# iSach/SoccerNeRFs

Measured on AMD Instinct MI355X. Metric: train rays/sec (K-Planes Broadcast-style, whole job), higher is better.
Workload: dtype bf16; 1 GPU; K-Planes default multiscale-res 1-16 on synthetic Broadcast-style (k-planes preset: 4096 rays/GPU/step, samples 256/128/64, 5 scales x 6 planes C=32, 156.0 M params), full train step incl. Adam; rays_per_gpu=4096, images=627, params=156049664, parallelism=single GPU

## Files before the change

include/snerf.h:

```cpp
#ifndef SNERF_H
#define SNERF_H

#include <stdint.h>

#ifdef __cplusplus
extern "C" {
#endif

typedef void* snerf_stream_t;

#define SNERF_OK 0
#define SNERF_ERR_ARG (-1)
#define SNERF_ERR_UNSUPPORTED (-2)

#define SNERF_MAX_SCALES 8
#define SNERF_ABI_VERSION 16
#define SNERF_ABI_REVISION 2

int snerf_abi_version(void);
int snerf_abi_revision(void);
const char* snerf_last_error(void);
const char* snerf_target_arch(void);

typedef struct {
// ... 221 lines not shown
} snerf_adam_dyn;
int snerf_adam_prepare(snerf_adam_dyn* dyn, float lr, float beta1, float beta2, int32_t policy, int32_t force_nonfinite, snerf_stream_t stream);

int snerf_adam_step(const float* p, float* p_out, float* g, float* m, float* v, int64_t n, float lr, float beta1, float beta2, float eps,
                    int32_t step, float grad_scale, int32_t zero_grad, snerf_adam_dyn* dyn, snerf_stream_t stream);

int snerf_adam_planes_step(const snerf_kplanes_desc* desc, const float* p_in, float* p_out, float* g, float* m, float* v,
                           float c_space_tv, float c_time_smooth, float c_sparse, float* losses, int32_t n_slots, float lr, float beta1,
                           float beta2, float eps, int32_t step, float grad_scale, int32_t zero_grad, snerf_adam_dyn* dyn,
                           snerf_stream_t stream);

int snerf_adam_planes_step_range(const snerf_kplanes_desc* desc, const float* p_in, float* p_out, float* g, float* m, float* v,
                                 float c_space_tv, float c_time_smooth, float c_sparse, float* losses, int32_t n_slots, float lr, float beta1,
                                 float beta2, float eps, int32_t step, float grad_scale, int32_t zero_grad, int64_t range_lo, int64_t range_hi,
                                 snerf_adam_dyn* dyn, snerf_stream_t stream);

#define SNERF_COMM_ID_BYTES 128
int snerf_comm_unique_id(void* id128);
int snerf_comm_create(int32_t world, int32_t rank, const void* id128, void** comm_out);
int snerf_comm_destroy(void* comm);
int snerf_allreduce_grads(void* comm, float* grads, int64_t n, snerf_stream_t stream);


typedef struct {
  const int64_t* indices;
  const float* fx; const float* fy; const float* cx; const float* cy;
  const float* c2w;
  const float* cam_times;
  int32_t R;
  int32_t collide;
// ... 152 lines not shown
                                float* target, snerf_stream_t stream);

int snerf_sample_pixels_sphere(const float* u, int32_t R, int32_t M, int32_t H, int32_t W, const uint8_t* images, int64_t* indices,
                               float* target, snerf_stream_t stream);

int snerf_mask_pack(const uint8_t* mask, int64_t n_pixels, int64_t first_pixel, int64_t count, uint32_t* bits, int32_t* block_counts,
                    snerf_stream_t stream);

int snerf_sample_pixels_masked(const float* u, int32_t R, int32_t M, int32_t H, int32_t W, const uint32_t* bits, const int64_t* block_prefix,
                               int64_t n_blocks, const uint8_t* images, int64_t* indices, float* target, snerf_stream_t stream);

int snerf_sort_rays_by_key(const int64_t* indices_in, const int32_t* image_key, int32_t n_keys, int32_t R, const float* aux_in, int32_t aux_cols,
                           int64_t* indices_out, float* aux_out, snerf_stream_t stream);

int snerf_ray_time_order(const float* times, int32_t R, int32_t* order_out, snerf_stream_t stream);

int snerf_aabb_collide(const float* origins, const float* dirs, int32_t R, const float* aabb6, float near_plane, int32_t training,
                       float* nears, float* fars, snerf_stream_t stream);

typedef struct {
  int32_t D;
  int32_t C;
  int32_t L;
  int32_t grid_C;
  int32_t H;
  int32_t gridtype;
  int32_t align_corners;
  float S;
  int32_t offsets[33];
} snerf_tgrid_desc;
// ... 142 lines not shown
```

soccernerfs_amd/_lib.py:

```python
import ctypes as C
import os

import torch

_PKG = os.path.dirname(os.path.abspath(__file__))
LIB_PATH = os.path.join(_PKG, "libsnerf.so")

MAX_SCALES = 8
ABI_VERSION = 16
ABI_REVISION = 2


class KPlanesDesc(C.Structure):
    _c_struct_ = "snerf_kplanes_desc"
    _fields_ = [
        ("n_scales", C.c_int32),
        ("C", C.c_int32),
        ("concat", C.c_int32),
        ("n_coords", C.c_int32),
        ("res", (C.c_int32 * 4) * MAX_SCALES),
        ("off", (C.c_int64 * 6) * MAX_SCALES),
    ]


# ... 30 lines not shown
    _c_struct_ = "snerf_mlp_desc"
    _fields_ = [("d_in", C.c_int32), ("hidden", C.c_int32), ("n_hidden", C.c_int32), ("d_out", C.c_int32),
                ("hidden_act", C.c_int32), ("out_act", C.c_int32), ("operands", C.c_int32)]


class DensityBwdLevel(C.Structure):
    _c_struct_ = "snerf_density_bwd_level"
    _fields_ = [("desc", C.c_void_p), ("planes", C.c_void_p), ("coords", C.c_void_p), ("N", C.c_int64), ("net", C.c_void_p), ("W", C.c_void_p),
                ("gdens", C.c_void_p), ("grad_planes", C.c_void_p), ("workspace", C.c_void_p), ("gX", C.c_void_p)]


class AdamDyn(C.Structure):
    _c_struct_ = "snerf_adam_dyn"
    _fields_ = [("nonfinite", C.c_int32), ("t", C.c_int32), ("skipped", C.c_int32), ("dropped", C.c_int32),
                ("step_size", C.c_float), ("inv_sqrt_bc2", C.c_float), ("skip", C.c_int32), ("_pad", C.c_int32)]


class RenderArgs(C.Structure):
    _c_struct_ = "snerf_render_args"
    _fields_ = [("weights", C.c_void_p), ("rgb", C.c_void_p), ("ebins", C.c_void_p), ("bg", C.c_void_p),
                ("R", C.c_int32), ("S", C.c_int32), ("bg_mode", C.c_int32), ("training", C.c_int32),
                ("rgb_out", C.c_void_p), ("acc_out", C.c_void_p), ("depth_median", C.c_void_p), ("depth_expected", C.c_void_p),
                ("median_rgb", C.c_void_p), ("median_index", C.c_void_p)]


class RayTrainArgs(C.Structure):
    _c_struct_ = "snerf_ray_train_args"
    _fields_ = [("density", C.c_void_p), ("ebins", C.c_void_p), ("sbins", C.c_void_p), ("rgb", C.c_void_p), ("bg", C.c_void_p), ("target", C.c_void_p),
                ("R", C.c_int32), ("S", C.c_int32), ("bg_mode", C.c_int32), ("go_scale", C.c_float), ("dist_scale", C.c_float),
                ("weights", C.c_void_p), ("rgb_out", C.c_void_p), ("acc_out", C.c_void_p), ("depth_median", C.c_void_p), ("sqerr_rays", C.c_void_p),
# ... 120 lines not shown
    "snerf_kplanes_density_bwd": "s:PIP",
    "snerf_kplanes_density_bwd_budget": "s:PIIP",
    "snerf_render_fwd": "s:PP",
    "snerf_ray_train_fwd_bwd": "s:PP",
    "snerf_render_bwd": "s:PPPIPPIIPPIP",
    "snerf_render_mse_bwd": "s:PPPIPPFIIPPPP",
    "snerf_distortion": "s:PPIIFPPIP",
    "snerf_interlevel": "s:PPIPPIIFPPP",
    "snerf_depth_loss": "s:PPPPFIIFPPIP",
    "snerf_urf_depth_loss": "s:PPPPPFIIFPPPIP",
    "snerf_plane_reg": "s:PPPFFFPIIP",
    "snerf_adam_prepare": "s:PFFFIIP",
    "snerf_adam_step": "s:PPPPPLFFFFIFIPP",
    "snerf_adam_planes_step": "s:PPPPPPFFFPIFFFFIFIPP",
    "snerf_adam_planes_step_range": "s:PPPPPPFFFPIFFFFIFILLPP",
    "snerf_comm_unique_id": "s:P",
    "snerf_comm_create": "s:IIPP",
    "snerf_comm_destroy": "s:P",
    "snerf_allreduce_grads": "s:PPLP",
    "snerf_raygen": "s:PP",
    "snerf_raygen_frame": "s:PP",
    "snerf_raygen_lens": "s:PP",
    "snerf_raygen_frame_lens": "s:PP",
    "snerf_raygen_cam": "s:PP",
    "snerf_raygen_frame_cam": "s:PP",
    "snerf_pose_apply": "s:PPPIIPP",
    "snerf_raygen_pose_bwd": "s:PP",
    "snerf_sample_pixels_uniform": "s:PIIIIPPPP",
    "snerf_sample_pixels_sphere": "s:PIIIIPPPP",
    "snerf_mask_pack": "s:PLLLPPP",
    "snerf_sample_pixels_masked": "s:PIIIIPPLPPPP",
    "snerf_sort_rays_by_key": "s:PPIIPIPPP",
    "snerf_ray_time_order": "s:PIPP",
    "snerf_aabb_collide": "s:PPIPFIPPP",
    "snerf_tgrid_encode_fwd": "s:PPPPPILPP",
    "snerf_tgrid_encode_fwd_dydx": "s:PPPPPILPPP",
    "snerf_tgrid_input_bwd": "s:PPLIIIPP",
    "snerf_tgrid_encode_bwd": "s:PPPPILPPP",
    "snerf_tgrid_encode_bwd_fx": "s:PPPPILPPP",
    "snerf_tgrid_tile_plan_make": "s:PLIIP",
    "snerf_tgrid_bwd_bin": "s:PPPPILPPPPPP",
    "snerf_tgrid_bwd_tiles": "s:PPLPPPPPP",
    "snerf_tgrid_bwd_tiles_adam": "s:PPLPPPPPPPPFFFFIIIPP",
    "snerf_tgrid_encode_bwd_levels": "s:PPPPILPPIIP",
    "snerf_tgrid_tv_fwd": "s:PLIIIPIP",
    "snerf_tgrid_tv_bwd": "s:PLIIIPPP",
    "snerf_tgrid_tv_fwd_bwd": "s:PLIIIFPIPP",
    "snerf_tgrid_tv_sign": "s:PLIIIFPIPP",
# ... 92 lines not shown
```

soccernerfs_amd/csrc/optim.hip:

```cpp
#include "plane_adam_common.hpp"

namespace snerf {

__global__ void adam_prepare_kernel(snerf_adam_dyn* dyn, float lr, float b1, float b2, int policy, int force_nonfinite) {
  if (threadIdx.x != 0 || blockIdx.x != 0) return;
  const int nf = dyn->nonfinite | force_nonfinite;
  const int skip = (policy == 1 && nf) ? 1 : 0;
  dyn->nonfinite = 0;
  dyn->skip = skip;
  if (skip) { dyn->skipped += 1; return; }
  const int t = dyn->t + 1;
  dyn->t = t;
  const double bc1 = 1.0 - pow((double)b1, (double)t), bc2 = 1.0 - pow((double)b2, (double)t);
  dyn->step_size = (float)((double)lr / bc1);
  dyn->inv_sqrt_bc2 = (float)(1.0 / sqrt(bc2));
}

template <int C, bool ADAM>
__global__ __launch_bounds__(256) void plane_reg_kernel(RegArgs a) {
  int s = 0, p = 0;
  const int blk = (int)blockIdx.x + a.blk_base;
  {
    const int b = blk;
    bool found = false;
    for (int ss = a.d.n_scales - 1; ss >= 0 && !found; --ss)
      for (int pp = a.n_planes - 1; pp >= 0; --pp)
        if (b >= a.blk_off[ss][pp]) { s = ss; p = pp; found = true; break; }
  }
  int ax, bx;
  plane_axes(a.n_planes, p, ax, bx);
  const int W = a.d.res[s][ax], H = a.d.res[s][bx];
  const bool time_plane = (a.n_planes == 6) && (bx == 3);
  constexpr int C4 = C / 4;
  const uint32_t n4 = (uint32_t)H * (uint32_t)W * C4;
  const uint32_t e = (uint32_t)(blk - a.blk_off[s][p]) * 256u + threadIdx.x;
  float l_tv = 0.f, l_sm = 0.f, l_l1 = 0.f;
// ... 32 lines not shown
        *reinterpret_cast<float4*>(gp) = add4(old, g);
      }
    }
  }
  __shared__ float red[3][4];
  l_tv = wave_sum(l_tv); l_sm = wave_sum(l_sm); l_l1 = wave_sum(l_l1);
  const int wv = threadIdx.x >> 6, lane = threadIdx.x & 63;
  if (lane == 0) { red[0][wv] = l_tv; red[1][wv] = l_sm; red[2][wv] = l_l1; }
  __syncthreads();
  if (threadIdx.x < 3 && a.losses) {
    float v = red[threadIdx.x][0] + red[threadIdx.x][1] + red[threadIdx.x][2] + red[threadIdx.x][3];
    if (v != 0.f) atomicAdd(a.losses + (size_t)(blk % a.n_slots) * 16 + threadIdx.x, v);
  }
}

__global__ __launch_bounds__(256) void adam_kernel(const float* p, float* p_out, float* __restrict__ g, float* __restrict__ m, float* __restrict__ v,
                                                  int64_t n, float step_size_h, float b1, float b2, float inv_sqrt_bc2_h, float eps,
                                                  float grad_scale, int zero_grad, snerf_adam_dyn* dyn) {
  const int64_t n4 = n / 4;
  const int64_t i = (int64_t)blockIdx.x * blockDim.x + threadIdx.x;
  const DynConsts dc = load_dyn(dyn, step_size_h, inv_sqrt_bc2_h);
  const float step_size = dc.step_size, inv_sqrt_bc2 = dc.inv_sqrt_bc2;
  if (dc.skip) {
    if (i < n4) {
      if (p_out != p) stnt4(p_out + i * 4, ldnt4(p + i * 4));
      if (zero_grad) stnt4(g + i * 4, make_float4(0.f, 0.f, 0.f, 0.f));
    }
    if (blockIdx.x == 0 && threadIdx.x < (n & 3)) {
      const int64_t j = n4 * 4 + threadIdx.x;
      p_out[j] = p[j];
      if (zero_grad) g[j] = 0.f;
    }
    return;
  }
  if (i < n4) {
    float4 pp = ldnt4(p + i * 4), gg = ldnt4(g + i * 4), mm = ldnt4(m + i * 4), vv = ldnt4(v + i * 4);
    float* P = &pp.x; float* G = &gg.x; float* M = &mm.x; float* V = &vv.x;
    int ndrop = 0;
#pragma unroll
    for (int k = 0; k < 4; ++k) {
      float gk = G[k] * grad_scale;
      if (!(fabsf(gk) <= 3.402823466e+38f)) { gk = 0.f; ++ndrop; }
      M[k] = b1 * M[k] + (1.f - b1) * gk;
      V[k] = b2 * V[k] + (1.f - b2) * gk * gk;
      float denom = sqrtf(V[k]) * inv_sqrt_bc2 + eps;
      P[k] = P[k] - step_size * (M[k] / denom);
    }
    if (ndrop && dyn) atomicAdd(&dyn->dropped, ndrop);
    stnt4(p_out + i * 4, pp);
    stnt4(m + i * 4, mm);
    stnt4(v + i * 4, vv);
    if (zero_grad && (gg.x != 0.f || gg.y != 0.f || gg.z != 0.f || gg.w != 0.f)) stnt4(g + i * 4, make_float4(0.f, 0.f, 0.f, 0.f));
  }
  if (blockIdx.x == 0 && threadIdx.x < (n & 3)) {
    int64_t i = n4 * 4 + threadIdx.x;
    float gk = g[i] * grad_scale;
    if (!(fabsf(gk) <= 3.402823466e+38f)) { gk = 0.f; if (dyn) atomicAdd(&dyn->dropped, 1); }
    float mk = b1 * m[i] + (1.f - b1) * gk;
    float vk = b2 * v[i] + (1.f - b2) * gk * gk;
    m[i] = mk; v[i] = vk;
    p_out[i] = p[i] - step_size * (mk / (sqrtf(vk) * inv_sqrt_bc2 + eps));
    if (zero_grad) g[i] = 0.f;
  }
}

__global__ __launch_bounds__(256) void adam_tv_kernel(float* p, float* __restrict__ g, float* __restrict__ m, float* __restrict__ v, int64_t n, float step_size_h,
                                                     float b1, float b2, float inv_sqrt_bc2_h, float eps, float grad_scale, int zero_grad, int grid_C, int col_a,
                                                     int col_b, const float* __restrict__ srow, snerf_adam_dyn* dyn) {
  const int64_t n4 = n / 4;
  const int64_t i = (int64_t)blockIdx.x * blockDim.x + threadIdx.x;
  if (i >= n4) return;
  const DynConsts dc = load_dyn(dyn, step_size_h, inv_sqrt_bc2_h);
  const float step_size = dc.step_size, inv_sqrt_bc2 = dc.inv_sqrt_bc2;
  if (dc.skip) {
    if (zero_grad) stnt4(g + i * 4, make_float4(0.f, 0.f, 0.f, 0.f));
    return;
  }
// ... 106 lines not shown
  if (desc->C == 32) hipLaunchKernelGGL((plane_reg_kernel<32, true>), dim3(grid), dim3(256), 0, st, a);
  else if (desc->C == 16) hipLaunchKernelGGL((plane_reg_kernel<16, true>), dim3(grid), dim3(256), 0, st, a);
  else hipLaunchKernelGGL((plane_reg_kernel<8, true>), dim3(grid), dim3(256), 0, st, a);
  SNERF_LAUNCH_CHECK("adam_planes_step");
  return 0;
}

extern "C" int snerf_adam_planes_step(const snerf_kplanes_desc* desc, const float* p_in, float* p_out, float* g, float* m, float* v,
                                      float c_space_tv, float c_time_smooth, float c_sparse, float* losses, int32_t n_slots, float lr, float beta1,
                                      float beta2, float eps, int32_t step, float grad_scale, int32_t zero_grad, snerf_adam_dyn* dyn,
                                      snerf_stream_t stream) {
  return snerf_adam_planes_step_range(desc, p_in, p_out, g, m, v, c_space_tv, c_time_smooth, c_sparse, losses, n_slots, lr, beta1, beta2, eps, step,
                                      grad_scale, zero_grad, 0, INT64_MAX & ~(int64_t)3, dyn, stream);
}

extern "C" int snerf_adam_step_tv(float* p, float* g, float* m, float* v, int64_t rows, int32_t grid_C, int32_t col_a, int32_t col_b, const float* srow,
                                  float lr, float beta1, float beta2, float eps, int32_t step, float grad_scale, int32_t zero_grad, snerf_adam_dyn* dyn,
                                  snerf_stream_t stream) {
  SNERF_REQUIRE(rows >= 1 && grid_C >= 4 && (step >= 1 || dyn), "adam_step_tv: rows=%lld grid_C=%d step=%d", (long long)rows, grid_C, step);
  SNERF_REQUIRE(col_a >= 0 && col_a < grid_C && col_b >= 0 && col_b < grid_C && col_a != col_b, "adam_step_tv: columns (%d, %d) of %d", col_a, col_b, grid_C);
  SNERF_REQUIRE(p && g && m && v && srow, "adam_step_tv: null buffer");
  const int64_t n = rows * grid_C;
  SNERF_REQUIRE((n & 3) == 0, "adam_step_tv: rows * grid_C = %lld must be a multiple of 4", (long long)n);
  SNERF_REQUIRE((((uintptr_t)p | (uintptr_t)g | (uintptr_t)m | (uintptr_t)v) & 15) == 0, "adam_step_tv: buffers must be 16-byte aligned");
  float step_size = 0.f, inv_sqrt_bc2 = 0.f;
  if (!dyn) adam_consts(lr, beta1, beta2, step, step_size, inv_sqrt_bc2);
  const int64_t blocks = (n / 4 + 255) / 256;
  SNERF_REQUIRE(blocks < (1LL << 31), "adam_step_tv: table too large for one launch");
  hipLaunchKernelGGL(adam_tv_kernel, dim3((unsigned)blocks), dim3(256), 0, (hipStream_t)stream, p, g, m, v, n, step_size, beta1, beta2, inv_sqrt_bc2, eps,
                     grad_scale, zero_grad, grid_C, col_a, col_b, srow, dyn);
// ... 30 lines not shown
```

soccernerfs_amd/csrc/raygen.hip:

```cpp
#include "raygen_common.hpp"

#pragma clang fp contract(off)

namespace snerf {

struct RaygenArgs {
  const int64_t* indices;
  const float* fx; const float* fy; const float* cx; const float* cy;
  const float* c2w;
  const float* cam_times;
  int R;
  float* origins; float* dirs; float* pixel_area; float* dir_norm; float* times;
  int collide; int training; float near_plane;
  float aabb_min[3], aabb_max[3];
  float* nears; float* fars;
};

__global__ void raygen_kernel(RaygenArgs a) {
  int r = blockIdx.x * blockDim.x + threadIdx.x;
  if (r >= a.R) return;
  const int64_t c = a.indices[(int64_t)r * 3], yi = a.indices[(int64_t)r * 3 + 1], xi = a.indices[(int64_t)r * 3 + 2];
  const PixelRay p = pixel_ray(yi, xi, a.fx[c], a.fy[c], a.cx[c], a.cy[c], a.c2w + c * 12);
#pragma unroll
  for (int k = 0; k < 3; ++k) { a.origins[(int64_t)r * 3 + k] = p.o[k]; a.dirs[(int64_t)r * 3 + k] = p.d[k]; }
// ... 112 lines not shown
  for (int i = threadIdx.x; i < n_pow2; i += blockDim.x)
    s_tk[i] = i < R ? (((uint64_t)__float_as_uint(times[i]) << 32) | (uint32_t)i) : ~0ull;
  __syncthreads();
  for (int k = 2; k <= n_pow2; k <<= 1)
    for (int lj = 31 - __clz(k >> 1); lj >= 0; --lj) {
      const int j = 1 << lj;
      for (int t = threadIdx.x; t < n_pow2 / 2; t += blockDim.x) {
        const int i = ((t >> lj) << (lj + 1)) | (t & (j - 1)), l = i + j;
        const bool up = (i & k) == 0;
        const uint64_t a = s_tk[i], b = s_tk[l];
        if ((a > b) == up) { s_tk[i] = b; s_tk[l] = a; }
      }
      __syncthreads();
    }
  for (int r = threadIdx.x; r < R; r += blockDim.x) order_out[r] = (int32_t)(uint32_t)s_tk[r];
}

__global__ void aabb_kernel(const float* __restrict__ o, const float* __restrict__ d, int R, float near_plane, int training, const float* amin3,
                            float* __restrict__ nears, float* __restrict__ fars, float a0, float a1, float a2, float b0, float b1, float b2) {
  int r = blockIdx.x * blockDim.x + threadIdx.x;
  if (r >= R) return;
  const float mn[3] = {a0, a1, a2}, mx[3] = {b0, b1, b2};
  float tn = -INFINITY, tf = INFINITY;
#pragma unroll
  for (int k = 0; k < 3; ++k) {
    float inv = 1.f / (d[(int64_t)r * 3 + k] + 1e-6f);
    float t1 = (mn[k] - o[(int64_t)r * 3 + k]) * inv, t2 = (mx[k] - o[(int64_t)r * 3 + k]) * inv;
    tn = fmaxf(tn, fminf(t1, t2));
    tf = fminf(tf, fmaxf(t1, t2));
  }
// ... 214 lines not shown
extern "C" int snerf_sort_rays_by_key(const int64_t* indices_in, const int32_t* image_key, int32_t n_keys, int32_t R, const float* aux_in,
                                      int32_t aux_cols, int64_t* indices_out, float* aux_out, snerf_stream_t stream) {
  SNERF_REQUIRE(R >= 0 && R <= 16384 && n_keys >= 1 && n_keys <= (1 << 18) && aux_cols >= 0,
                "sort_rays_by_key: R=%d (<= 16384) n_keys=%d (<= 262144) aux_cols=%d", R, n_keys, aux_cols);
  if (R == 0) return 0;
  SNERF_REQUIRE(indices_in && image_key && indices_out && indices_in != indices_out && (aux_cols == 0 || (aux_in && aux_out && aux_in != aux_out)),
                "sort_rays_by_key: null or aliased buffer (the sort is out of place)");
  int n = 2;
  while (n < R) n <<= 1;
  hipLaunchKernelGGL(sort_rays_kernel, dim3(1), dim3(256), (size_t)n * sizeof(uint32_t), (hipStream_t)stream, indices_in, image_key, R, n, aux_in, aux_cols,
                     indices_out, aux_out);
  SNERF_LAUNCH_CHECK("sort_rays_by_key");
  return 0;
}

extern "C" int snerf_ray_time_order(const float* times, int32_t R, int32_t* order_out, snerf_stream_t stream) {
  SNERF_REQUIRE(R >= 0 && R <= 16384, "ray_time_order: R=%d (<= 16384: one workgroup sorts in LDS)", R);
  if (R == 0) return 0;
  SNERF_REQUIRE(times && order_out, "ray_time_order: null buffer");
  int n = 2;
  while (n < R) n <<= 1;
  SNERF_ALLOW_LDS(ray_time_order_kernel, 16384 * (int)sizeof(uint64_t));
  hipLaunchKernelGGL(ray_time_order_kernel, dim3(1), dim3(256), (size_t)n * sizeof(uint64_t), (hipStream_t)stream, times, R, n, order_out);
  SNERF_LAUNCH_CHECK("ray_time_order");
  return 0;
}

extern "C" int snerf_aabb_collide(const float* origins, const float* dirs, int32_t R, const float* aabb6, float near_plane, int32_t training,
                                  float* nears, float* fars, snerf_stream_t stream) {
  SNERF_REQUIRE(R >= 0 && aabb6, "aabb_collide: bad arguments");
  if (R == 0) return 0;
  SNERF_REQUIRE(origins && dirs && nears && fars, "aabb_collide: null buffer");
  hipLaunchKernelGGL(aabb_kernel, dim3(ceil_div(R, 256)), dim3(256), 0, (hipStream_t)stream, origins, dirs, R, near_plane, training, nullptr, nears,
                     fars, aabb6[0], aabb6[1], aabb6[2], aabb6[3], aabb6[4], aabb6[5]);
  SNERF_LAUNCH_CHECK("aabb_collide");
  return 0;
}

extern "C" int snerf_pose_apply(const float* c2w, const float* pose_adjustment, const int32_t* group, int32_t M, int32_t G, float* c2w_adj,
                                snerf_stream_t stream) {
// ... 32 lines not shown
```

soccernerfs_amd/ops.py:

```python
import ctypes as C

from typing import Optional

import torch

from . import _lib
from .plane_set import PlaneSet


def _stream():
    return C.c_void_p(torch.cuda.current_stream().cuda_stream)


def _ptr(t: torch.Tensor):
    return C.c_void_p(t.data_ptr())


def _f32c(t: torch.Tensor, name: str) -> torch.Tensor:
    if not t.is_cuda:
        raise RuntimeError(f"{name}: expected a HIP device tensor (the HIP library is the only product path)")
    if t.dtype != torch.float32:
        raise RuntimeError(f"{name}: expected float32, got {t.dtype}")
    return t.contiguous()

# ... 828 lines not shown
    R = indices.shape[0]
    if R > 16384 or R == 0:
        return (indices, aux) if aux is not None else indices
    if not indices.is_cuda or indices.dtype != torch.int64 or image_key.dtype != torch.int32 or not image_key.is_cuda:
        raise RuntimeError("sort_rays_by_time: indices must be an int64 HIP tensor [R,3] and image_key an int32 HIP tensor")
    indices = indices.contiguous()
    out = torch.empty_like(indices)
    aux_c = _f32c(aux, "sort_rays_by_time aux").reshape(R, -1) if aux is not None else None
    aux_out = torch.empty_like(aux_c) if aux_c is not None else None
    _lib.call("sort_rays_by_key", _ptr(indices), _ptr(image_key), n_keys, R, _ptr(aux_c) if aux_c is not None else None,
              aux_c.shape[1] if aux_c is not None else 0, _ptr(out), _ptr(aux_out) if aux_out is not None else None,
              _stream())
    return (out, aux_out.view(aux.shape)) if aux is not None else out


def ray_time_order(times: torch.Tensor, out: Optional[torch.Tensor] = None) -> torch.Tensor:
    times = _f32c(times, "times").reshape(-1)
    R = times.numel()
    if out is None:
        out = torch.empty(R, dtype=torch.int32, device=times.device)
    if not out.is_cuda or out.dtype != torch.int32 or not out.is_contiguous() or out.numel() < R:
        raise RuntimeError("ray_time_order: out must be a contiguous int32 HIP tensor of at least R elements")
    _lib.call("ray_time_order", _ptr(times), R, _ptr(out), _stream())
    return out[:R]


def sample_pixels_uniform(u: torch.Tensor, num_images: int, height: int, width: int, images: Optional[torch.Tensor] = None):
    u = _f32c(u, "u")
    R = u.shape[0]
    idx = torch.empty(R, 3, dtype=torch.int64, device=u.device)
    target = None
    if images is not None:
        if not images.is_cuda or images.dtype != torch.uint8 or not images.is_contiguous() or tuple(images.shape) != (num_images, height, width, 3):
            raise RuntimeError("sample_pixels_uniform: images must be a contiguous uint8 HIP tensor [M,H,W,3]")
        target = torch.empty(R, 3, dtype=torch.float32, device=u.device)
    _lib.call("sample_pixels_uniform", _ptr(u), R, num_images, height, width, _ptr(images) if images is not None else None, _ptr(idx),
              _ptr(target) if target is not None else None, _stream())
    return idx, target
# ... 111 lines not shown
```

soccernerfs_amd/trainer.py:

```python
import ctypes as C
from dataclasses import dataclass, field
from typing import Dict, List, Optional, Sequence, Tuple

import torch

from . import _lib, ops
from .fused_step import FusedStep, _On, _align4, anneal_value, cosine_lr_factor, update_schedule
from .streams import side_stream
from .plane_set import PlaneSet
from .tcnn_compat import Network


@dataclass
class KPlanesTrainConfig:

    aabb_scale: float = 1.5
    spacetime_resolution: Sequence[int] = (64, 64, 64, 100)
    multiscale_res: Sequence[int] = (1, 2, 4, 8, 16)
    feature_dim: int = 32
    proposal_resolutions: Sequence[Sequence[int]] = ((128, 128, 128, 100), (256, 256, 256, 100))
    proposal_feature_dim: int = 8
    sigma_net_hidden_dim: int = 128
    rgb_net_hidden_dim: int = 64
    disable_viewing_dependent: bool = True
# ... 34 lines not shown
    mlp_grad_workspace: bool = True
    interleave_proposal_levels: bool = False
    fix_capacity: Optional[int] = None
    exchange_chunks: int = 2
    grad_transport: str = "fp32"
    param_transport: str = "fp32"
    emulate_transports: str = ""
    deterministic: bool = False
    nonfinite_policy: str = "skip_step"
    fused_field: bool = True
    quotient_scatter: bool = True
    quotient_epilogue: bool = True
    fused_proposal: bool = True
    fused_proposal_backward: bool = True
    proposal_backward_workgroups_per_cu: float = 1.0
    pass_b_beside_head: bool = True
    sort_before_field_fwd: bool = False
    field_fwd_time_order: bool = True
    pipeline_sweep: str = ""
    ray_gradients: bool = False
    freeze_time_planes: bool = False
    freeze_space_planes: bool = False


class KPlanesTrainer(FusedStep):

    def __init__(self, cfg: KPlanesTrainConfig, num_rays: int, device="cuda:0", process_group=None):
        self.cfg, self.R, self.dev = cfg, num_rays, torch.device(device)
        self.pg = process_group
        self.world = torch.distributed.get_world_size(process_group) if process_group is not None else 1
# ... 159 lines not shown
        self.pass_b_beside_head = cfg.pass_b_beside_head
        self._in_train_step = False
        self.fused_proposal = bool(cfg.fused_proposal and all(self.lib.snerf_kplanes_density_fwd_supported(C.byref(dp), C.byref(net.desc))
                                                             for dp, net in zip(self._desc_prop, self.prop_nets)))
        self._keep_pfeat = True
        self.fused_proposal_backward = bool(cfg.fused_proposal_backward and self.fused_proposal and not cfg.deterministic
                                            and all(f"prop{i}.mlp" in self._mlp_ws for i in range(len(self.prop_nets)))
                                            and all(self.lib.snerf_kplanes_density_bwd_supported(C.byref(dp), C.byref(net.desc))
                                                    for dp, net in zip(self._desc_prop, self.prop_nets)))
        if cfg.proposal_backward_workgroups_per_cu < 0:
            raise ValueError(f"proposal_backward_workgroups_per_cu={cfg.proposal_backward_workgroups_per_cu} (0 = uncapped, or workgroups per CU)")
        self._prop_bwd_workgroups = 0
        if cfg.proposal_backward_workgroups_per_cu > 0 and self.fused_proposal_backward:
            cus = torch.cuda.get_device_properties(self.dev).multi_processor_count
            self._prop_bwd_workgroups = max(1, int(round(cfg.proposal_backward_workgroups_per_cu * cus)))
        if self.world > 1:
            self._plan_exchange()

    @torch.no_grad()
    def _sync_frozen_halves(self):
        if self._frozen:
            self._params_alt.copy_(self.params)

    def _plain_adam_ranges(self):
        if not self._frozen:
            return [(0, self.n_proposal_params, "proposal_networks"), (self.n_proposal_params, self.n_params, "fields")]
        out = []
        sets = [(f"prop{i}.planes", ps, "proposal_networks") for i, ps in enumerate(self.prop_planes)] + [("field.planes", self.field_planes, "fields")]
        for name, ps, g in sets:
            o = self.off[name][0]
# ... 424 lines not shown
                proposal_chain(after=main.record_event())
        if not overlap:
            self._proposal_backward(proposal_grads)
        self._prop_pending = None
        for st in joins:
            if defer_prop_join and not sharded and st is self._side.get("prop"):
                self._prop_pending = st
            else:
                main.wait_stream(st)
        if cfg.ray_gradients:
            self._ray_gradient(self._desc_field, self.field_planes.planes, self._coords[2], R * self.S[2], b["gfeat"])
        self._reduce_mlp_grads(("field.sigma", "field.color"))
        if self._prop_pending is None:
            self._reduce_mlp_grads(("prop0.mlp", "prop1.mlp"))

    def _join_prop(self):
        if self._prop_pending is not None:
            torch.cuda.current_stream().wait_stream(self._prop_pending)
            self._prop_pending = None
            self._reduce_mlp_grads(("prop0.mlp", "prop1.mlp"))

    def loss_dict(self) -> Dict[str, torch.Tensor]:
        b, co, R = self.buf, self.cfg.loss_coefficients, self.R
        self._join_prop()
        if self._reg_work is not None:
            self._reg_work.wait()
        if self._field_adam_done is not None:
            torch.cuda.current_stream().wait_event(self._field_adam_done)
        d = dict(self.last)
        d["rgb_loss"] = b["sqerr"].sum() / (3 * R) * co["rgb_loss"]
        d["distortion_loss"] = b["dist_rays"].mean() * co["distortion_loss"]
        d["interlevel_loss"] = (b["inter_rays"][0].sum() + b["inter_rays"][1].sum()) / (R * self.S[2]) * co["interlevel_loss"]
        reg = b["reg"][:, :, :3].sum(1)
        d["space_tv_loss"], d["time_smoothness_loss"], d["sparse_transients_loss"] = (
            reg[0, 0] * co["space_tv_loss"], reg[0, 1] * co["time_smoothness_loss"], reg[0, 2] * co["sparse_transients_loss"])
# ... 166 lines not shown
        self._reg_work = sdist.all_reduce_sum_(self.buf["reg"][0], self.pg, async_op=True)
        self._params_alt = self.params
        self._repoint(new)
        self._finish_step()

    def _adam_mlps(self, new, off, lr, gs):
        with self._span("adam_step.mlps"):
            o0, n0 = off["field.sigma"]
            o1, n1 = off["field.color"]
            dyn_f, dyn_p = self._dyn["fields"], self._dyn["proposal_networks"]
            for (o, n), dyn in ((off["prop0.mlp"], dyn_p), (off["prop1.mlp"], dyn_p), ((o0, o1 + n1 - o0), dyn_f)):
                n4 = _align4(n)
                ops.adam_step(self.params[o:o + n4], self.grads[o:o + n4], self.exp_avg[o:o + n4], self.exp_avg_sq[o:o + n4], self.step + 1, lr,
                              eps=self.cfg.adam_eps, grad_scale=gs, zero_grad=True, p_out=new[o:o + n4], dyn=dyn)

    def _finest_offset(self) -> int:
        return int(self._desc_field.off[len(self.cfg.multiscale_res) - 1][0])

    def _adam_field_range(self, lo: int, hi: Optional[int], side: bool, role: str = "adam", span: str = "adam_planes.field", after=None):
        cfg, co = self.cfg, self.cfg.loss_coefficients
        lr = cfg.lr * cosine_lr_factor(self.step, cfg.warm_up_end, cfg.max_steps, cfg.lr_alpha)
        n4 = _align4(self.field_planes.numel)
        rng_ = (lo, n4 if hi is None else hi)
        o, n = self.off["field.planes"]
        args = (self.field_planes, self.params[o:o + n], self._params_alt[o:o + n], self.gviews["field.planes"], self.mviews["field.planes"],
                self.vviews["field.planes"], tuple(co[k] for k in ("space_tv_loss", "time_smoothness_loss", "sparse_transients_loss")),
                self.buf["reg"][0], self.step + 1, lr)
        self._prepare_group("fields", lr)
        kw = dict(eps=cfg.adam_eps, grad_scale=self._grad_scale, zero_grad=True, shard_range=rng_, dyn=self._dyn["fields"], desc=self._desc_field)
        if not side:
# ... 27 lines not shown
        if self.grads_fx is not None:
            self._join_prop()
            self._convert_fx()
        if not fused_reg:
            self._join_prop()
            self._prepare_group("fields", lr)
            self._prepare_group("proposal_networks", lr)
            with self._span("adam_step"):
                for lo, hi, g in self._plain_adam_ranges():
                    ops.adam_step(self.params[lo:hi], self.grads[lo:hi], self.exp_avg[lo:hi], self.exp_avg_sq[lo:hi], self.step + 1, lr, eps=cfg.adam_eps,
                                  grad_scale=gs, zero_grad=True, dyn=self._dyn[g])
            self._finish_step()
            return
        new = self._params_alt
        off = self.off
        sl = lambda t, name: t[off[name][0]:off[name][0] + off[name][1]]
        async_field = self.async_field_adam and self.overlap
        if not self._reg_zeroed:
            self.buf["reg"].zero_()
        emu = self.cfg.emulate_transports if self.world == 1 else ""
        if emu in ("grad", "both"):
            gv = self.gviews["field.planes"]
            gv.copy_(gv.to(torch.bfloat16))
        if async_field and self._passb_fine_done is not None:
            cut = self._finest_offset()
            ev, fine_first = self._passb_fine_done
            first, second = ((cut, None), (0, cut)) if fine_first else ((0, cut), (cut, None))
            names = ("adam_planes.field.fine", "adam_planes.field.coarse") if fine_first else ("adam_planes.field.coarse", "adam_planes.field.fine")
            self._adam_field_range(*first, side=True, role="sort", after=ev, span=names[0])
            fine_done = self._stream("sort").record_event()
            self._adam_field_range(*second, side=True, span=names[1])
            self._stream("adam").wait_event(fine_done)
            self._passb_fine_done = None
            self.field_sweep_launches = 2
        else:
            self._passb_fine_done = None
            self._adam_field_range(0, None, side=async_field)
            self.field_sweep_launches = 1
        if emu in ("param", "both"):
            o_, n_ = self.off["field.planes"]
            with _On(self, self._stream("adam") if async_field else torch.cuda.current_stream()):
                old_, new_ = self.params[o_:o_ + n_], self._params_alt[o_:o_ + n_]
                new_.copy_(old_ + (new_ - old_).to(torch.bfloat16).float())
        if async_field:
            self._field_adam_done = self._stream("adam").record_event()
        self._reg_zeroed = False
        self._join_prop()
        self._prepare_group("fields", lr)
        self._prepare_group("proposal_networks", lr)
        sets = [(f"prop{i}.planes", self.prop_planes[i], ("space_tv_proposal_loss", "time_smoothness_proposal_loss",
                                                          "sparse_transients_proposal_loss"), 1 + i) for i in range(2)]
        for name, ps, keys, row in sets:
            with self._span("adam_planes." + name.split(".")[0]):
                ops.adam_planes_step(ps, sl(self.params, name), sl(new, name), self.gviews[name], self.mviews[name], self.vviews[name],
                                     tuple(co[k] for k in keys), self.buf["reg"][row], self.step + 1, lr, eps=cfg.adam_eps, grad_scale=gs,
                                     dyn=self._dyn["proposal_networks"], desc=self._desc_prop[row - 1])
        self._adam_mlps(new, off, lr, gs)
        self._params_alt = self.params
        self._repoint(new)
        self._finish_step()

    def random_draws(self) -> Dict[str, torch.Tensor]:
        R, (S0, S1, S2) = self.R, self.S
        sj = self.cfg.use_single_jitter
        c0, c1, c2 = (1, 1, 1) if sj else (S0 + 1, S1 + 1, S2 + 1)
        flat = torch.rand(R * (c0 + c1 + c2 + 3), device=self.dev)
        o = 0
        out = []
        for c in (c0, c1, c2, 3):
            out.append(flat[o:o + R * c].view(R, c))
            o += R * c
        return {"t_rand": out[0], "u": [out[1], out[2]], "bg": out[3]}

    def train_step(self, rays: Dict[str, torch.Tensor], target: torch.Tensor, rng: Optional[Dict[str, torch.Tensor]] = None,
                   depth: Optional[torch.Tensor] = None):
# ... 109 lines not shown
```

Measured before the change: 2.166 million rays/s.

## Fuse proposal-plane and MLP Adam updates into one segmented launch; rank-based ray time order

Adds a segmented Adam kernel that updates both proposal plane sets (with their regularizer terms) and the flat MLP parameter ranges in a single launch. It also folds the replicated MLP gradient workspace into the gradient inside the Adam pass instead of running a separate reduction. Separately, the single-workgroup bitonic sort for ray time ordering is replaced with a multi-workgroup counting-rank kernel. The aim is to cut kernel launch count and serial tail work in the optimizer phase. The cost is more complex segment bookkeeping and O(R^2) comparisons for the ranking.

```diff
diff --git a/include/snerf.h b/include/snerf.h
--- a/include/snerf.h
+++ b/include/snerf.h
@@ -259,6 +259,26 @@
                                  float c_space_tv, float c_time_smooth, float c_sparse, float* losses, int32_t n_slots, float lr, float beta1,
                                  float beta2, float eps, int32_t step, float grad_scale, int32_t zero_grad, int64_t range_lo, int64_t range_hi,
                                  snerf_adam_dyn* dyn, snerf_stream_t stream);
+
+typedef struct {
+  int32_t kind;
+  int32_t n_slots;
+  const snerf_kplanes_desc* desc;
+  const float* p_in;
+  float* p_out;
+  float* g;
+  float* m;
+  float* v;
+  float c_space_tv, c_time_smooth, c_sparse;
+  int32_t _pad;
+  float* losses;
+  int64_t n;
+  snerf_adam_dyn* dyn;
+  const snerf_mlp_desc* net;
+  float* workspace;
+} snerf_adam_segment;
+int snerf_adam_segments_step(const snerf_adam_segment* segs, int32_t n_segs, float lr, float beta1, float beta2, float eps, int32_t step,
+                             float grad_scale, int32_t zero_grad, snerf_stream_t stream);
 
 #define SNERF_COMM_ID_BYTES 128
 int snerf_comm_unique_id(void* id128);
@@ -441,6 +461,7 @@
                            int64_t* indices_out, float* aux_out, snerf_stream_t stream);
 
 int snerf_ray_time_order(const float* times, int32_t R, int32_t* order_out, snerf_stream_t stream);
+int snerf_ray_time_order_reference(const float* times, int32_t R, int32_t* order_out, snerf_stream_t stream);
 
 int snerf_aabb_collide(const float* origins, const float* dirs, int32_t R, const float* aabb6, float near_plane, int32_t training,
                        float* nears, float* fars, snerf_stream_t stream);
diff --git a/soccernerfs_amd/_lib.py b/soccernerfs_amd/_lib.py
--- a/soccernerfs_amd/_lib.py
+++ b/soccernerfs_amd/_lib.py
@@ -68,6 +68,13 @@
     _c_struct_ = "snerf_adam_dyn"
     _fields_ = [("nonfinite", C.c_int32), ("t", C.c_int32), ("skipped", C.c_int32), ("dropped", C.c_int32),
                 ("step_size", C.c_float), ("inv_sqrt_bc2", C.c_float), ("skip", C.c_int32), ("_pad", C.c_int32)]
+
+
+class AdamSegment(C.Structure):
+    _c_struct_ = "snerf_adam_segment"
+    _fields_ = [("kind", C.c_int32), ("n_slots", C.c_int32), ("desc", C.c_void_p), ("p_in", C.c_void_p), ("p_out", C.c_void_p), ("g", C.c_void_p),
+                ("m", C.c_void_p), ("v", C.c_void_p), ("c_space_tv", C.c_float), ("c_time_smooth", C.c_float), ("c_sparse", C.c_float),
+                ("_pad", C.c_int32), ("losses", C.c_void_p), ("n", C.c_int64), ("dyn", C.c_void_p), ("net", C.c_void_p), ("workspace", C.c_void_p)]
 
 
 class RenderArgs(C.Structure):
@@ -218,6 +225,7 @@
     "snerf_adam_step": "s:PPPPPLFFFFIFIPP",
     "snerf_adam_planes_step": "s:PPPPPPFFFPIFFFFIFIPP",
     "snerf_adam_planes_step_range": "s:PPPPPPFFFPIFFFFIFILLPP",
+    "snerf_adam_segments_step": "s:PIFFFFIFIP",
     "snerf_comm_unique_id": "s:P",
     "snerf_comm_create": "s:IIPP",
     "snerf_comm_destroy": "s:P",
@@ -236,6 +244,7 @@
     "snerf_sample_pixels_masked": "s:PIIIIPPLPPPP",
     "snerf_sort_rays_by_key": "s:PPIIPIPPP",
     "snerf_ray_time_order": "s:PIPP",
+    "snerf_ray_time_order_reference": "s:PIPP",
     "snerf_aabb_collide": "s:PPIPFIPPP",
     "snerf_tgrid_encode_fwd": "s:PPPPPILPP",
     "snerf_tgrid_encode_fwd_dydx": "s:PPPPPILPPP",
diff --git a/soccernerfs_amd/csrc/optim.hip b/soccernerfs_amd/csrc/optim.hip
--- a/soccernerfs_amd/csrc/optim.hip
+++ b/soccernerfs_amd/csrc/optim.hip
@@ -1,3 +1,4 @@
+#include "mlp_args.hpp"
 #include "plane_adam_common.hpp"
 
 namespace snerf {
@@ -17,9 +18,8 @@
 }
 
 template <int C, bool ADAM>
-__global__ __launch_bounds__(256) void plane_reg_kernel(RegArgs a) {
+__device__ __forceinline__ void plane_reg_block(const RegArgs& a, const int blk) {
   int s = 0, p = 0;
-  const int blk = (int)blockIdx.x + a.blk_base;
   {
     const int b = blk;
     bool found = false;
@@ -82,22 +82,52 @@
   }
 }
 
-__global__ __launch_bounds__(256) void adam_kernel(const float* p, float* p_out, float* __restrict__ g, float* __restrict__ m, float* __restrict__ v,
-                                                  int64_t n, float step_size_h, float b1, float b2, float inv_sqrt_bc2_h, float eps,
-                                                  float grad_scale, int zero_grad, snerf_adam_dyn* dyn) {
+template <int C, bool ADAM>
+__global__ __launch_bounds__(256) void plane_reg_kernel(RegArgs a) {
+  plane_reg_block<C, ADAM>(a, (int)blockIdx.x + a.blk_base);
+}
+
+struct FlatFold { float* ws; int64_t ws_stride, n_fold; int reps; };
+template <bool FOLD>
+__device__ __forceinline__ float fold_gw(const FlatFold& f, int64_t e, float g, bool& folded) {
+  if (!FOLD || e >= f.n_fold) return g;
+  float s = 0.f;
+  for (int k = 0; k < f.reps; ++k) {
+    s += f.ws[k * f.ws_stride + e];
+    f.ws[k * f.ws_stride + e] = 0.f;
+  }
+  if (s != 0.f) { g = g + s; folded = true; }
+  return g;
+}
+
+template <bool FOLD>
+__device__ __forceinline__ void adam_flat_block(const float* p, float* p_out, float* __restrict__ g, float* __restrict__ m, float* __restrict__ v,
+                                                int64_t n, float step_size_h, float b1, float b2, float inv_sqrt_bc2_h, float eps, float grad_scale,
+                                                int zero_grad, snerf_adam_dyn* dyn, const FlatFold& fold, const int64_t blk) {
   const int64_t n4 = n / 4;
-  const int64_t i = (int64_t)blockIdx.x * blockDim.x + threadIdx.x;
+  const int64_t i = blk * blockDim.x + threadIdx.x;
   const DynConsts dc = load_dyn(dyn, step_size_h, inv_sqrt_bc2_h);
   const float step_size = dc.step_size, inv_sqrt_bc2 = dc.inv_sqrt_bc2;
   if (dc.skip) {
     if (i < n4) {
       if (p_out != p) stnt4(p_out + i * 4, ldnt4(p + i * 4));
+      if (FOLD && i * 4 < fold.n_fold) {
+        float4 gg = ldnt4(g + i * 4);
+        float* G = &gg.x;
+        bool folded = false;
+#pragma unroll
+        for (int k = 0; k < 4; ++k) G[k] = fold_gw<FOLD>(fold, i * 4 + k, G[k], folded);
+        if (!zero_grad && folded) stnt4(g + i * 4, gg);
+      }
       if (zero_grad) stnt4(g + i * 4, make_float4(0.f, 0.f, 0.f, 0.f));
     }
-    if (blockIdx.x == 0 && threadIdx.x < (n & 3)) {
+    if (blk == 0 && threadIdx.x < (n & 3)) {
       const int64_t j = n4 * 4 + threadIdx.x;
       p_out[j] = p[j];
+      bool folded = false;
+      const float gj = fold_gw<FOLD>(fold, j, g[j], folded);
       if (zero_grad) g[j] = 0.f;
+      else if (folded) g[j] = gj;
     }
     return;
   }
@@ -105,8 +135,10 @@
     float4 pp = ldnt4(p + i * 4), gg = ldnt4(g + i * 4), mm = ldnt4(m + i * 4), vv = ldnt4(v + i * 4);
     float* P = &pp.x; float* G = &gg.x; float* M = &mm.x; float* V = &vv.x;
     int ndrop = 0;
+    bool folded = false;
 #pragma unroll
     for (int k = 0; k < 4; ++k) {
+      G[k] = fold_gw<FOLD>(fold, i * 4 + k, G[k], folded);
       float gk = G[k] * grad_scale;
       if (!(fabsf(gk) <= 3.402823466e+38f)) { gk = 0.f; ++ndrop; }
       M[k] = b1 * M[k] + (1.f - b1) * gk;
@@ -119,16 +151,57 @@
     stnt4(m + i * 4, mm);
     stnt4(v + i * 4, vv);
     if (zero_grad && (gg.x != 0.f || gg.y != 0.f || gg.z != 0.f || gg.w != 0.f)) stnt4(g + i * 4, make_float4(0.f, 0.f, 0.f, 0.f));
-  }
-  if (blockIdx.x == 0 && threadIdx.x < (n & 3)) {
+    else if (FOLD && folded) stnt4(g + i * 4, gg);
+  }
+  if (blk == 0 && threadIdx.x < (n & 3)) {
     int64_t i = n4 * 4 + threadIdx.x;
-    float gk = g[i] * grad_scale;
+    bool folded = false;
+    const float gi = fold_gw<FOLD>(fold, i, g[i], folded);
+    float gk = gi * grad_scale;
     if (!(fabsf(gk) <= 3.402823466e+38f)) { gk = 0.f; if (dyn) atomicAdd(&dyn->dropped, 1); }
     float mk = b1 * m[i] + (1.f - b1) * gk;
     float vk = b2 * v[i] + (1.f - b2) * gk * gk;
     m[i] = mk; v[i] = vk;
     p_out[i] = p[i] - step_size * (mk / (sqrtf(vk) * inv_sqrt_bc2 + eps));
     if (zero_grad) g[i] = 0.f;
+    else if (folded) g[i] = gi;
+  }
+}
+
+__global__ __launch_bounds__(256) void adam_kernel(const float* p, float* p_out, float* __restrict__ g, float* __restrict__ m, float* __restrict__ v,
+                                                  int64_t n, float step_size_h, float b1, float b2, float inv_sqrt_bc2_h, float eps,
+                                                  float grad_scale, int zero_grad, snerf_adam_dyn* dyn) {
+  adam_flat_block<false>(p, p_out, g, m, v, n, step_size_h, b1, b2, inv_sqrt_bc2_h, eps, grad_scale, zero_grad, dyn, FlatFold{}, (int64_t)blockIdx.x);
+}
+
+constexpr int SEG_PLANE_SETS = 2, SEG_FLAT = 4;
+struct FlatSeg {
+  const float* p; float* p_out; float* g; float* m; float* v;
+  int64_t n;
+  snerf_adam_dyn* dyn;
+  FlatFold fold;
+};
+struct SegArgs {
+  RegArgs plane[SEG_PLANE_SETS];
+  FlatSeg flat[SEG_FLAT];
+  int first[SEG_PLANE_SETS + SEG_FLAT];
+  int n_plane, n_flat;
+  float step_size, b1, b2, inv_sqrt_bc2, eps, grad_scale;
+  int zero_grad;
+};
+
+template <int C>
+__global__ __launch_bounds__(256) void adam_segments_kernel(SegArgs a) {
+  const int b = (int)blockIdx.x;
+  int seg = 0;
+  for (int k = 1; k < a.n_plane + a.n_flat; ++k)
+    if (b >= a.first[k]) seg = k;
+  if (seg < a.n_plane) {
+    plane_reg_block<C, true>(a.plane[seg], b - a.first[seg]);
+  } else {
+    const FlatSeg& f = a.flat[seg - a.n_plane];
+    adam_flat_block<true>(f.p, f.p_out, f.g, f.m, f.v, f.n, a.step_size, a.b1, a.b2, a.inv_sqrt_bc2, a.eps, a.grad_scale, a.zero_grad, f.dyn, f.fold,
+                          (int64_t)(b - a.first[seg]));
   }
 }
 
@@ -265,6 +338,79 @@
                                       grad_scale, zero_grad, 0, INT64_MAX & ~(int64_t)3, dyn, stream);
 }
 
+extern "C" int snerf_adam_segments_step(const snerf_adam_segment* segs, int32_t n_segs, float lr, float beta1, float beta2, float eps, int32_t step,
+                                        float grad_scale, int32_t zero_grad, snerf_stream_t stream) {
+  SNERF_REQUIRE(segs && n_segs >= 1 && n_segs <= SEG_PLANE_SETS + SEG_FLAT, "adam_segments_step: %d segments (1..%d)", n_segs, SEG_PLANE_SETS + SEG_FLAT);
+  SegArgs a = {};
+  a.b1 = beta1; a.b2 = beta2; a.eps = eps; a.grad_scale = grad_scale; a.zero_grad = zero_grad;
+  int C = 0;
+  bool need_step = false;
+  int64_t grid[SEG_PLANE_SETS + SEG_FLAT];
+  int64_t plane_blocks[SEG_PLANE_SETS];
+  for (int k = 0; k < n_segs; ++k) {
+    const snerf_adam_segment& g = segs[k];
+    SNERF_REQUIRE(g.kind == 0 || g.kind == 1, "adam_segments_step: segment %d has kind %d (0 flat, 1 plane set)", k, g.kind);
+    SNERF_REQUIRE(g.p_in && g.p_out && g.g && g.m && g.v, "adam_segments_step: segment %d: null buffer", k);
+    need_step = need_step || !g.dyn;
+    if (g.kind == 1) {
+      const snerf_kplanes_desc* desc = g.desc;
+      SNERF_REQUIRE(a.n_plane < SEG_PLANE_SETS, "adam_segments_step: more than %d plane sets", SEG_PLANE_SETS);
+      SNERF_REQUIRE(desc && g.p_in != g.p_out, "adam_segments_step: segment %d: a plane set needs its descriptor and ping-pong parameters (p_in != p_out)", k);
+      SNERF_REQUIRE(desc->n_scales >= 1 && desc->n_scales <= SNERF_MAX_SCALES, "adam_segments_step: n_scales=%d", desc->n_scales);
+      SNERF_REQUIRE(desc->C == 8 || desc->C == 16 || desc->C == 32, "adam_segments_step: C=%d unsupported", desc->C);
+      SNERF_REQUIRE(C == 0 || C == desc->C, "adam_segments_step: the plane sets of one call share a channel count (%d, %d)", C, desc->C);
+      SNERF_REQUIRE(desc->n_coords == 3 || desc->n_coords == 4, "adam_segments_step: n_coords=%d", desc->n_coords);
+      SNERF_REQUIRE(!g.losses || g.n_slots >= 1, "adam_segments_step: n_slots=%d", g.n_slots);
+      C = desc->C;
+      RegArgs& r = a.plane[a.n_plane];
+      r.d = *desc;
+      r.n_planes = desc->n_coords == 4 ? 6 : 3;
+      r.planes = g.p_in; r.grad = g.g; r.c_tv = g.c_space_tv; r.c_smooth = g.c_time_smooth; r.c_l1 = g.c_sparse; r.losses = g.losses; r.n_slots = g.n_slots;
+      r.p_out = g.p_out; r.m = g.m; r.v = g.v; r.b1 = beta1; r.b2 = beta2; r.eps = eps; r.grad_scale = grad_scale; r.zero_grad = zero_grad;
+      r.range_lo = 0; r.range_hi = INT64_MAX & ~(int64_t)3; r.dyn = g.dyn; r.blk_base = 0;
+      int64_t blocks = 0;
+      for (int sc = 0; sc < desc->n_scales; ++sc)
+        for (int pl = 0; pl < r.n_planes; ++pl) {
+          int ax, bx;
+          plane_axes(r.n_planes, pl, ax, bx);
+          r.blk_off[sc][pl] = (int)blocks;
+          blocks += ((int64_t)desc->res[sc][ax] * desc->res[sc][bx] * (desc->C / 4) + 255) / 256;
+        }
+      plane_blocks[a.n_plane++] = blocks;
+    } else {
+      SNERF_REQUIRE(a.n_flat < SEG_FLAT, "adam_segments_step: more than %d flat segments", SEG_FLAT);
+      SNERF_REQUIRE(g.n >= 1, "adam_segments_step: segment %d: n=%lld", k, (long long)g.n);
+      SNERF_REQUIRE((((uintptr_t)g.p_in | (uintptr_t)g.p_out | (uintptr_t)g.g | (uintptr_t)g.m | (uintptr_t)g.v) & 15) == 0,
+                    "adam_segments_step: segment %d: buffers must be 16-byte aligned", k);
+      FlatSeg& f = a.flat[a.n_flat];
+      f.p = g.p_in; f.p_out = g.p_out; f.g = g.g; f.m = g.m; f.v = g.v; f.n = g.n; f.dyn = g.dyn;
+      if (g.net || g.workspace) {
+        SNERF_REQUIRE(g.net && g.workspace, "adam_segments_step: segment %d: a workspace to fold needs its MLP descriptor, and the other way round", k);
+        const int64_t n_fold = snerf_mlp_param_count(g.net);
+        SNERF_REQUIRE(n_fold > 0 && n_fold <= g.n, "adam_segments_step: segment %d: the net has %lld weights, the segment %lld floats", k, (long long)n_fold,
+                      (long long)g.n);
+        f.fold.ws = g.workspace; f.fold.ws_stride = gw_ws_stride(g.net); f.fold.n_fold = n_fold; f.fold.reps = GW_REPLICAS;
+      }
+      grid[SEG_PLANE_SETS + a.n_flat++] = ((g.n + 3) / 4 + 255) / 256;
+    }
+  }
+  SNERF_REQUIRE(!need_step || step >= 1, "adam_segments_step: step=%d (1-based) for a segment without device-side state", step);
+  if (need_step) adam_consts(lr, beta1, beta2, step, a.step_size, a.inv_sqrt_bc2);
+  for (int k = 0; k < a.n_plane; ++k) { a.plane[k].step_size = a.step_size; a.plane[k].inv_sqrt_bc2 = a.inv_sqrt_bc2; }
+  int64_t blocks = 0;
+  for (int k = 0; k < a.n_plane + a.n_flat; ++k) {
+    a.first[k] = (int)blocks;
+    blocks += k < a.n_plane ? plane_blocks[k] : grid[SEG_PLANE_SETS + k - a.n_plane];
+    SNERF_REQUIRE(blocks < (1LL << 31), "adam_segments_step: too many workgroups");
+  }
+  hipStream_t st = (hipStream_t)stream;
+  if (C == 32) hipLaunchKernelGGL((adam_segments_kernel<32>), dim3((unsigned)blocks), dim3(256), 0, st, a);
+  else if (C == 16) hipLaunchKernelGGL((adam_segments_kernel<16>), dim3((unsigned)blocks), dim3(256), 0, st, a);
+  else hipLaunchKernelGGL((adam_segments_kernel<8>), dim3((unsigned)blocks), dim3(256), 0, st, a);
+  SNERF_LAUNCH_CHECK("adam_segments_step");
+  return 0;
+}
+
 extern "C" int snerf_adam_step_tv(float* p, float* g, float* m, float* v, int64_t rows, int32_t grid_C, int32_t col_a, int32_t col_b, const float* srow,
                                   float lr, float beta1, float beta2, float eps, int32_t step, float grad_scale, int32_t zero_grad, snerf_adam_dyn* dyn,
                                   snerf_stream_t stream) {
diff --git a/soccernerfs_amd/csrc/raygen.hip b/soccernerfs_amd/csrc/raygen.hip
--- a/soccernerfs_amd/csrc/raygen.hip
+++ b/soccernerfs_amd/csrc/raygen.hip
@@ -150,6 +150,33 @@
       __syncthreads();
     }
   for (int r = threadIdx.x; r < R; r += blockDim.x) order_out[r] = (int32_t)(uint32_t)s_tk[r];
+}
+
+constexpr int RANK_RAYS = 32, RANK_PARTS = 256 / RANK_RAYS;
+__global__ __launch_bounds__(256) void ray_time_rank_kernel(const float* __restrict__ times, int R, int chunk, int32_t* __restrict__ order_out) {
+  extern __shared__ __align__(16) uint32_t s_tb[];
+  const int n_pad = RANK_PARTS * chunk;
+  uint32_t* s_cnt = s_tb + n_pad;
+  for (int i = threadIdx.x; i < n_pad; i += blockDim.x) s_tb[i] = i < R ? __float_as_uint(times[i]) : 0xffffffffu;
+  __syncthreads();
+  const int lane = threadIdx.x % RANK_RAYS, part = threadIdx.x / RANK_RAYS;
+  const int ray = blockIdx.x * RANK_RAYS + lane;
+  const uint64_t mine = ((uint64_t)s_tb[ray < R ? ray : 0] << 32) | (uint32_t)ray;
+  uint32_t cnt = 0;
+  const int j0 = part * chunk;
+  for (int j = j0; j < j0 + chunk; j += 4) {
+    const uint4 tb = *reinterpret_cast<const uint4*>(s_tb + j);
+    cnt += ((((uint64_t)tb.x << 32) | (uint32_t)j) < mine) + ((((uint64_t)tb.y << 32) | (uint32_t)(j + 1)) < mine) +
+           ((((uint64_t)tb.z << 32) | (uint32_t)(j + 2)) < mine) + ((((uint64_t)tb.w << 32) | (uint32_t)(j + 3)) < mine);
+  }
+  s_cnt[part * RANK_RAYS + lane] = cnt;
+  __syncthreads();
+  if (part == 0 && ray < R) {
+    uint32_t rank = 0;
+#pragma unroll
+    for (int p = 0; p < RANK_PARTS; ++p) rank += s_cnt[p * RANK_RAYS + lane];
+    order_out[rank] = ray;
+  }
 }
 
 __global__ void aabb_kernel(const float* __restrict__ o, const float* __restrict__ d, int R, float near_plane, int training, const float* amin3,
@@ -394,16 +421,32 @@
   return 0;
 }
 
-extern "C" int snerf_ray_time_order(const float* times, int32_t R, int32_t* order_out, snerf_stream_t stream) {
-  SNERF_REQUIRE(R >= 0 && R <= 16384, "ray_time_order: R=%d (<= 16384: one workgroup sorts in LDS)", R);
-  if (R == 0) return 0;
-  SNERF_REQUIRE(times && order_out, "ray_time_order: null buffer");
+static int ray_time_order_bitonic(const float* times, int32_t R, int32_t* order_out, snerf_stream_t stream) {
   int n = 2;
   while (n < R) n <<= 1;
   SNERF_ALLOW_LDS(ray_time_order_kernel, 16384 * (int)sizeof(uint64_t));
   hipLaunchKernelGGL(ray_time_order_kernel, dim3(1), dim3(256), (size_t)n * sizeof(uint64_t), (hipStream_t)stream, times, R, n, order_out);
   SNERF_LAUNCH_CHECK("ray_time_order");
   return 0;
+}
+
+extern "C" int snerf_ray_time_order(const float* times, int32_t R, int32_t* order_out, snerf_stream_t stream) {
+  SNERF_REQUIRE(R >= 0 && R <= 16384, "ray_time_order: R=%d (<= 16384: every workgroup holds all times in LDS)", R);
+  if (R == 0) return 0;
+  SNERF_REQUIRE(times && order_out, "ray_time_order: null buffer");
+  const int chunk = ceil_div(ceil_div(R, RANK_PARTS), 4) * 4;
+  const int lds_bytes = (RANK_PARTS * chunk + RANK_PARTS * RANK_RAYS) * (int)sizeof(uint32_t);
+  SNERF_ALLOW_LDS(ray_time_rank_kernel, (16384 + RANK_PARTS * RANK_RAYS) * (int)sizeof(uint32_t));
+  hipLaunchKernelGGL(ray_time_rank_kernel, dim3(ceil_div(R, RANK_RAYS)), dim3(256), (size_t)lds_bytes, (hipStream_t)stream, times, R, chunk, order_out);
+  SNERF_LAUNCH_CHECK("ray_time_order");
+  return 0;
+}
+
+extern "C" int snerf_ray_time_order_reference(const float* times, int32_t R, int32_t* order_out, snerf_stream_t stream) {
+  SNERF_REQUIRE(R >= 0 && R <= 16384, "ray_time_order_reference: R=%d (<= 16384: one workgroup sorts in LDS)", R);
+  if (R == 0) return 0;
+  SNERF_REQUIRE(times && order_out, "ray_time_order_reference: null buffer");
+  return ray_time_order_bitonic(times, R, order_out, stream);
 }
 
 extern "C" int snerf_aabb_collide(const float* origins, const float* dirs, int32_t R, const float* aabb6, float near_plane, int32_t training,
diff --git a/soccernerfs_amd/ops.py b/soccernerfs_amd/ops.py
--- a/soccernerfs_amd/ops.py
+++ b/soccernerfs_amd/ops.py
@@ -866,14 +866,14 @@
     return (out, aux_out.view(aux.shape)) if aux is not None else out
 
 
-def ray_time_order(times: torch.Tensor, out: Optional[torch.Tensor] = None) -> torch.Tensor:
+def ray_time_order(times: torch.Tensor, out: Optional[torch.Tensor] = None, reference: bool = False) -> torch.Tensor:
     times = _f32c(times, "times").reshape(-1)
     R = times.numel()
     if out is None:
         out = torch.empty(R, dtype=torch.int32, device=times.device)
     if not out.is_cuda or out.dtype != torch.int32 or not out.is_contiguous() or out.numel() < R:
         raise RuntimeError("ray_time_order: out must be a contiguous int32 HIP tensor of at least R elements")
-    _lib.call("ray_time_order", _ptr(times), R, _ptr(out), _stream())
+    _lib.call("ray_time_order_reference" if reference else "ray_time_order", _ptr(times), R, _ptr(out), _stream())
     return out[:R]
 
 
diff --git a/soccernerfs_amd/trainer.py b/soccernerfs_amd/trainer.py
--- a/soccernerfs_amd/trainer.py
+++ b/soccernerfs_amd/trainer.py
@@ -72,6 +72,7 @@
     fused_proposal: bool = True
     fused_proposal_backward: bool = True
     proposal_backward_workgroups_per_cu: float = 1.0
+    fused_small_adam: bool = True
     pass_b_beside_head: bool = True
     sort_before_field_fwd: bool = False
     field_fwd_time_order: bool = True
@@ -261,6 +262,9 @@
         if cfg.proposal_backward_workgroups_per_cu > 0 and self.fused_proposal_backward:
             cus = torch.cuda.get_device_properties(self.dev).multi_processor_count
             self._prop_bwd_workgroups = max(1, int(round(cfg.proposal_backward_workgroups_per_cu * cus)))
+        self.fused_small_adam = bool(cfg.fused_small_adam and self.world == 1 and self.grads_fx is None
+                                     and self._desc_prop[0].C == self._desc_prop[1].C and self._desc_prop[0].C in (8, 16, 32))
+        self._small_segments = (_lib.AdamSegment * 5)()
         if self.world > 1:
             self._plan_exchange()
 
@@ -715,11 +719,12 @@
         if self._prop_pending is None:
             self._reduce_mlp_grads(("prop0.mlp", "prop1.mlp"))
 
-    def _join_prop(self):
+    def _join_prop(self, reduce: bool = True):
         if self._prop_pending is not None:
             torch.cuda.current_stream().wait_stream(self._prop_pending)
             self._prop_pending = None
-            self._reduce_mlp_grads(("prop0.mlp", "prop1.mlp"))
+            if reduce:
+                self._reduce_mlp_grads(("prop0.mlp", "prop1.mlp"))
 
     def loss_dict(self) -> Dict[str, torch.Tensor]:
         b, co, R = self.buf, self.cfg.loss_coefficients, self.R
@@ -916,6 +921,31 @@
                 ops.adam_step(self.params[o:o + n4], self.grads[o:o + n4], self.exp_avg[o:o + n4], self.exp_avg_sq[o:o + n4], self.step + 1, lr,
                               eps=self.cfg.adam_eps, grad_scale=gs, zero_grad=True, p_out=new[o:o + n4], dyn=dyn)
 
+    def _adam_small(self, new, off, lr, gs):
+        cfg, co = self.cfg, self.cfg.loss_coefficients
+        segs = self._small_segments
+        dyn_f, dyn_p = self._dyn["fields"].data_ptr(), self._dyn["proposal_networks"].data_ptr()
+        at = lambda t, o: t.data_ptr() + 4 * o
+        coefs = tuple(co[k] for k in ("space_tv_proposal_loss", "time_smoothness_proposal_loss", "sparse_transients_proposal_loss"))
+        for i in range(2):
+            sg, (o, _) = segs[i], off[f"prop{i}.planes"]
+            sg.kind, sg.n_slots, sg.desc = 1, ops.REG_SLOTS, C.addressof(self._desc_prop[i])
+            sg.p_in, sg.p_out, sg.g, sg.m, sg.v = at(self.params, o), at(new, o), at(self.grads, o), at(self.exp_avg, o), at(self.exp_avg_sq, o)
+            sg.c_space_tv, sg.c_time_smooth, sg.c_sparse = coefs
+            sg.losses, sg.dyn, sg.n, sg.net, sg.workspace = self.buf["reg"][1 + i].data_ptr(), dyn_p, 0, None, None
+        o0, o1, n1 = off["field.sigma"][0], *off["field.color"]
+        flat = ((*off["prop0.mlp"], dyn_p, "prop0.mlp"), (*off["prop1.mlp"], dyn_p, "prop1.mlp"), (o0, o1 + n1 - o0, dyn_f, None))
+        for sg, (o, n, dyn, gname) in zip(segs[2:], flat):
+            sg.kind, sg.n_slots, sg.desc, sg.losses = 0, 0, None, None
+            sg.p_in, sg.p_out, sg.g, sg.m, sg.v = at(self.params, o), at(new, o), at(self.grads, o), at(self.exp_avg, o), at(self.exp_avg_sq, o)
+            sg.n, sg.dyn = _align4(n), dyn
+            fold = gname is not None and gname in self._ws_dirty
+            sg.net = C.addressof(self._mlp_nets[gname].desc) if fold else None
+            sg.workspace = self._mlp_ws[gname].data_ptr() if fold else None
+            self._ws_dirty.discard(gname)
+        with self._span("adam_small"):
+            self._call("adam_segments_step", segs, 5, lr, 0.9, 0.999, cfg.adam_eps, self.step + 1, gs, 1, self._st)
+
     def _finest_offset(self) -> int:
         return int(self._desc_field.off[len(self.cfg.multiscale_res) - 1][0])
 
@@ -973,7 +1003,6 @@
             return
         new = self._params_alt
         off = self.off
-        sl = lambda t, name: t[off[name][0]:off[name][0] + off[name][1]]
         async_field = self.async_field_adam and self.overlap
         if not self._reg_zeroed:
             self.buf["reg"].zero_()
@@ -1004,9 +1033,22 @@
         if async_field:
             self._field_adam_done = self._stream("adam").record_event()
         self._reg_zeroed = False
-        self._join_prop()
+        self._join_prop(reduce=not self.fused_small_adam)
         self._prepare_group("fields", lr)
         self._prepare_group("proposal_networks", lr)
+        if self.fused_small_adam:
+            self._st = C.c_void_p(torch.cuda.current_stream().cuda_stream)
+            self._adam_small(new, off, lr, gs)
+        else:
+            self._adam_small_launches(new, off, lr, gs)
+        self._params_alt = self.params
+        self._repoint(new)
+        self._finish_step()
+
+    def _adam_small_launches(self, new, off, lr, gs):
+        cfg, co = self.cfg, self.cfg.loss_coefficients
+        sl = lambda t, name: t[off[name][0]:off[name][0] + off[name][1]]
+        self._reduce_mlp_grads(("prop0.mlp", "prop1.mlp"))
         sets = [(f"prop{i}.planes", self.prop_planes[i], ("space_tv_proposal_loss", "time_smoothness_proposal_loss",
                                                           "sparse_transients_proposal_loss"), 1 + i) for i in range(2)]
         for name, ps, keys, row in sets:
@@ -1015,9 +1057,6 @@
                                      tuple(co[k] for k in keys), self.buf["reg"][row], self.step + 1, lr, eps=cfg.adam_eps, grad_scale=gs,
                                      dyn=self._dyn["proposal_networks"], desc=self._desc_prop[row - 1])
         self._adam_mlps(new, off, lr, gs)
-        self._params_alt = self.params
-        self._repoint(new)
-        self._finish_step()
 
     def random_draws(self) -> Dict[str, torch.Tensor]:
         R, (S0, S1, S2) = self.R, self.S
```

Measured after the change: 2.166 million rays/s (median of 2 runs). Within noise of the previous version (-0.0%).
